# mjoppich/tsxCount

Measured on AMD Instinct MI355X. Metric: k-mers/sec inserted, k=31, 1e9 synthetic k-mers, 1/2/4/8 GPU; --check pass, higher is better.
Workload: dtype u64

## Files before the change

### tsxcount_amd/csrc/tsx_kernels.h

```cpp
#pragma once
#include "tsx_device.h"

namespace tsx {

constexpr int NT = 256;
constexpr int TILE = 4096;
constexpr int HALO = 128;
constexpr int BATCH = 2048;
constexpr int PER_THREAD = BATCH / NT;
constexpr int DSLOTS = 4096;
constexpr int DPROBES = 8;

__device__ __forceinline__ bool is_nl(uint32_t b) { return b == (uint32_t)'\n'; }
__device__ __forceinline__ uint32_t base_code(uint32_t b) { return ((b >> 1) ^ (b >> 2)) & 3u; }

__device__ __forceinline__ void classify16(const uint4 v, bool prev_nl, uint32_t &nl16, uint32_t &le16,
                                           uint32_t &code32) {
    const uint32_t w[4] = {v.x, v.y, v.z, v.w};
    nl16 = 0; code32 = 0;
#pragma unroll
    for (int i = 0; i < 4; ++i) {
        const uint32_t t = ((w[i] >> 1) ^ (w[i] >> 2)) & 0x03030303u;
        const uint32_t x = t | (t >> 6);
        code32 |= ((x | (x >> 12)) & 0xFFu) << (8 * i);
// ... 228 lines not shown
                if (__ballot(valid) == 0ULL) continue;
                uint64_t x[WK];
                extract_kmer<WK>(s_codes, pp, p.top_mask, x);
                uint64_t xp[WK];
#pragma unroll
                for (int t = 0; t < WK; ++t) xp[t] = __shfl_up((unsigned long long)x[t], 1, 64);
                const bool prev_valid = __shfl_up((int)valid, 1, 64) != 0;
                const bool leader = valid && (lane == 0 || !prev_valid || !kmer_eq<WK>(x, xp));
                const unsigned long long bnd = __ballot(leader || !valid);
                const unsigned long long above = (lane == 63) ? 0ULL : (bnd >> (lane + 1));
                const uint32_t runlen = (above ? (uint32_t)__builtin_ctzll(above) : (uint32_t)(63 - lane)) + 1u;
                added += valid ? 1ULL : 0ULL;
                if (leader) {
                    hash_key<CANON, WK>(p, (const uint64_t *)s_lut, x, hk[j]);
                    uint32_t slot = (uint32_t)(mix64(hk[j][0] ^ (WK > 1 ? hk[j][WK - 1] : 0)) >> 40) & (DSLOTS - 1);
                    slot_of[j] = -2; direct_cnt[j] = runlen;
                    for (int pr = 0; pr < DPROBES; ++pr) {
                        const uint32_t old = atomicCAS(&s_dpos[slot], 0u, pp + 1u);
                        if (old == 0u) {
                            atomicAdd(&s_dcnt[slot], runlen);
                            slot_of[j] = (int)slot;
                            break;
                        }
                        uint64_t y[WK];
                        extract_kmer<WK>(s_codes, old - 1u, p.top_mask, y);
                        if (kmer_eq<WK>(x, y)) {
                            atomicAdd(&s_dcnt[slot], runlen);
                            slot_of[j] = -1;
                            break;
                        }
                        slot = (slot + 1) & (DSLOTS - 1);
                    }
                }
            }
            lds_barrier();
#pragma unroll
            for (int j = 0; j < PER_THREAD; ++j) {
                if (slot_of[j] == -1) continue;
                uint64_t d = direct_cnt[j];
                if (slot_of[j] >= 0) {
                    d = s_dcnt[slot_of[j]];
                    s_dcnt[slot_of[j]] = 0;
                    s_dpos[slot_of[j]] = 0;
                }
                insert_key<WK>(p, hk[j], d);
            }
            lds_barrier();
        }
    }
    for (int d = 32; d > 0; d >>= 1) added += __shfl_down(added, d, 64);
    if (lane == 0 && added) atomicAdd(&p.stats[ST_KMERS], added);
}

template <bool HOMOUT = false, bool BR = false>
__global__ __launch_bounds__(NT, 5) void strip_desc_kernel(TableParams p, const uint8_t *buf, uint64_t n, uint64_t own_end,
                                                           int head_open, const uint32_t *tile_line, uint64_t ntiles,
                                                           uint4 *desc, uint64_t desc_cap, unsigned long long *desc_cnt,
                                                           unsigned long long *kmer_sum, int long_desc,
                                                           unsigned long long *hom_out = nullptr,
                                                           const uint16_t *qmap = nullptr) {
    __shared__ uint64_t s_codes[(TILE + HALO) / 32 + 2];
    __shared__ uint64_t s_nl[(TILE + HALO) / 64 + 3];
    __shared__ uint64_t s_le[TILE / 64];
    __shared__ uint8_t s_lb[TILE / 16];
    __shared__ uint32_t s_wsum[NT / 64];
    const int tid = threadIdx.x, lane = tid & 63, wave = tid >> 6;
    if (tid < 3) s_nl[(TILE + HALO) / 64 + tid] = ~0ULL;
    if (tid < 2) s_codes[(TILE + HALO) / 32 + tid] = 0;
    unsigned long long added = 0;
    unsigned long long hacc = 0;
    const uint32_t k = (uint32_t)p.k;
    const uint32_t region = blockIdx.x * (NT / 64) + wave;
    uint4 *my = desc + (uint64_t)region * desc_cap * (long_desc ? 2u : 1u);
    uint32_t fill = 0;
    const uint64_t start_lim = min(own_end, (n >= k) ? n - k + 1 : 0ULL);
    const uint64_t lt = (1ULL << lane) - 1ULL;

    uint4 cur = make_uint4(0x0A0A0A0Au, 0x0A0A0A0Au, 0x0A0A0A0Au, 0x0A0A0A0Au), hcur = cur;
    bool cur_pnl = true;
    uint32_t cur_line = 0;
    if ((uint64_t)blockIdx.x < ntiles) {
        const uint64_t off = (uint64_t)blockIdx.x * TILE + (uint64_t)tid * 16;
        cur_line = tile_line[blockIdx.x];
        cur = load16(buf, off, n);
        cur_pnl = prev_is_nl(buf, off, n, head_open);
        if (tid < HALO / 16) hcur = load16(buf, (uint64_t)blockIdx.x * TILE + TILE + (uint64_t)tid * 16, n);
    }
    for (uint64_t tile = blockIdx.x; tile < ntiles; tile += gridDim.x) {
        const uint64_t base = tile * TILE;
        lds_barrier();
        {
            uint32_t nl, le, code;
            classify16(cur, cur_pnl, nl, le, code);
            if constexpr (BR) nl |= rule_bits16<BR>(p, qmap, cur, base + (uint64_t)tid * 16, n);
            reinterpret_cast<uint32_t *>(s_codes)[tid] = code;
            reinterpret_cast<uint16_t *>(s_nl)[tid] = (uint16_t)nl;
            reinterpret_cast<uint16_t *>(s_le)[tid] = (uint16_t)le;
            if (tid < HALO / 16) {
                uint32_t hnl, hle, hcode;
                classify16(hcur, false, hnl, hle, hcode);
                if constexpr (BR) hnl |= rule_bits16<BR>(p, qmap, hcur, base + TILE + (uint64_t)tid * 16, n);
                reinterpret_cast<uint32_t *>(s_codes)[TILE / 16 + tid] = hcode;
                reinterpret_cast<uint16_t *>(s_nl)[TILE / 16 + tid] = (uint16_t)hnl;
            }
            const uint32_t c = __popc(le);
            const uint32_t inc = wave_incl_scan(c);
            if (lane == 63) s_wsum[wave] = inc;
            lds_barrier();
            uint32_t woff = cur_line;
            for (int w = 0; w < wave; ++w) woff += s_wsum[w];
            s_lb[tid] = (uint8_t)((woff + inc - c) & 3u);
        }
        {
            const uint64_t nt = tile + gridDim.x;
            if (nt < ntiles) {
                const uint64_t off = nt * TILE + (uint64_t)tid * 16;
                cur_line = tile_line[nt];
                cur = load16(buf, off, n);
                cur_pnl = prev_is_nl(buf, off, n, head_open);
                if (tid < HALO / 16) hcur = load16(buf, nt * TILE + TILE + (uint64_t)tid * 16, n);
            }
        }
        lds_barrier();
        const uint32_t s0 = (uint32_t)tid * 16;
        const uint32_t *codes32 = reinterpret_cast<const uint32_t *>(s_codes);
        const uint32_t *nl32 = reinterpret_cast<const uint32_t *>(s_nl);
        uint64_t m;
        {
            const uint32_t w = (uint32_t)tid >> 1, sh = ((uint32_t)tid & 1u) * 16u;
            const uint32_t a0 = nl32[w], a1 = nl32[w + 1], a2 = nl32[w + 2];
            m = (uint64_t)__funnelshift_r(a0, a1, sh) | ((uint64_t)__funnelshift_r(a1, a2, sh) << 32);
        }
        uint64_t r = m;
        uint32_t span = 1;
        while (span * 2 <= k) { r |= r >> span; span *= 2; }
        if (span < k) r |= r >> (k - span);
        const uint32_t e16 = reinterpret_cast<const uint16_t *>(s_le)[tid];
        const uint32_t lb = s_lb[tid];
        uint32_t c0 = e16 << 1; c0 ^= c0 << 1; c0 ^= c0 << 2; c0 ^= c0 << 4; c0 ^= c0 << 8;
        uint32_t c1 = (e16 & c0) << 1; c1 ^= c1 << 1; c1 ^= c1 << 2; c1 ^= c1 << 4; c1 ^= c1 << 8;
        const uint32_t l0 = (lb & 1u) ? 0xFFFFu : 0u, l1 = (lb & 2u) ? 0xFFFFu : 0u;
        const uint32_t b0 = c0 ^ l0, b1 = c1 ^ l1 ^ (c0 & l0);
        const uint64_t g0 = base + s0;
        const uint32_t jmax = (start_lim > g0) ? (uint32_t)min((uint64_t)16, start_lim - g0) : 0u;
        const uint32_t nb1 = (p.line_mask & 2u) ? ~b1 : ~0u;
        uint32_t vm = ~(uint32_t)r & b0 & nb1 & ((1u << jmax) - 1u);
        added += (unsigned long long)__popc(vm);
        if constexpr (HOMOUT) {
            if (vm) {
                const uint32_t c0 = codes32[tid], c1 = codes32[tid + 1], c2 = codes32[tid + 2];
                const uint64_t lo = (uint64_t)c0 | ((uint64_t)c1 << 32), hi = c2;
                const uint64_t xl = lo ^ ((lo >> 2) | (hi << 62)), xh = hi ^ (hi >> 2);
                const uint64_t nl = (xl | (xl >> 1)) & 0x5555555555555555ULL, nh = (xh | (xh >> 1)) & 0x5555555555555555ULL;
                const bool core_ok = ((nl >> 30) & ((1ULL << (2u * (k - 16u))) - 1ULL)) == 0ULL;
              if (core_ok) {
                const uint32_t z = (uint32_t)nl & 0x3FFFFFFFu;
                const uint32_t a = z ? ((31u - (uint32_t)__clz((int)z)) >> 1) + 1u : 0u;
                const uint32_t s2 = 2u * (k - 1u);
                const uint32_t zz = (uint32_t)((nl >> s2) | (nh << (64u - s2))) & 0x3FFFFFFFu;
                const uint32_t b = zz ? (uint32_t)(__ffs((int)zz) - 1) >> 1 : 15u;
                const uint32_t homm = (a <= b) ? (((2u << b) - 1u) & ~((1u << a) - 1u)) & 0xFFFFu : 0u;
                hacc += (unsigned long long)__popc(vm & homm) << (16u * ((c0 >> 30) & 3u));
                vm &= ~homm;
              }
            }
        }
        if (!long_desc) {
            const unsigned long long hb = __ballot(vm != 0u);
            if (hb) {
                const uint32_t nbr = (uint32_t)(((hb << 1) >> lane) & 1ULL) << 16;
                if (vm) my[fill + (uint32_t)__builtin_popcountll(hb & lt)] = make_uint4(codes32[tid], codes32[tid + 1], codes32[tid + 2], vm | nbr);
                fill += (uint32_t)__builtin_popcountll(hb);
            }
        } else {
            const uint32_t v1 = __shfl_down(vm, 1, 64), v2 = __shfl_down(vm, 2, 64), v3 = __shfl_down(vm, 3, 64);
            const uint32_t vlo = vm | (v1 << 16), vhi = v2 | (v3 << 16);
            const bool has = (lane & 3) == 0 && (vlo | vhi) != 0u;
            const unsigned long long hb = __ballot(has);
            if (hb) {
                if (has) {
                    uint4 *o = my + (uint64_t)(fill + (uint32_t)__builtin_popcountll(hb & lt)) * 2u;
                    o[0] = make_uint4(codes32[tid], codes32[tid + 1], codes32[tid + 2], codes32[tid + 3]);
                    o[1] = make_uint4(codes32[tid + 4], codes32[tid + 5], vlo, vhi);
                }
                fill += (uint32_t)__builtin_popcountll(hb);
            }
        }
    }
    for (int d = 32; d > 0; d >>= 1) added += __shfl_down(added, d, 64);
    if (lane == 0) {
        if (added) atomicAdd(&p.stats[ST_KMERS], added);
        if (added && kmer_sum) atomicAdd(kmer_sum, added);
        desc_cnt[region] = fill;
    }
    if constexpr (HOMOUT) {
#pragma unroll
        for (int b = 0; b < 4; ++b) {
            unsigned long long t = (hacc >> (16 * b)) & 0xFFFFULL;
            for (int d = 32; d > 0; d >>= 1) t += __shfl_down(t, d, 64);
            if (lane == 0 && t && hom_out) atomicAdd(&hom_out[b], t);
        }
    }
}

template <bool CANON = false>
__global__ __launch_bounds__(NT, 4) void walk_log_kernel(TableParams p, const uint4 *desc, uint64_t desc_cap,
                                                         const unsigned long long *desc_cnt, uint32_t nregions,
                                                         uint64_t *log, uint64_t log_cap, unsigned long long *log_cnt,
                                                         uint32_t *hist, uint32_t hist_nb, uint32_t hist_shift,
                                                         uint64_t n_packed, int long_desc, int own_only,
                                                         unsigned long long *emit_sum) {
    constexpr int HOT_N = 8;
    __shared__ uint64_t s_hot_key[(NT / 64) * HOT_N];
    __shared__ uint32_t s_hot_cnt[(NT / 64) * HOT_N];
    __shared__ uint32_t s_hist[(NT / 64) * 512];
    __shared__ uint64_t s_roll[CANON ? 128 : 64];
    uint64_t *const s_mroll = s_roll + 64;
    __shared__ uint64_t s_homh[4];
    extern __shared__ uint64_t s_lut[];
    const int tid = threadIdx.x, lane = tid & 63, wave = tid >> 6;
    const int lut_words = p.groups * (1 << p.g);
    for (int i = tid; i < lut_words; i += NT) s_lut[i] = p.lut[i];
    for (int i = tid; i < (NT / 64) * 512; i += NT) s_hist[i] = 0;
    if (tid < 64) s_roll[tid] = p.roll[tid];
    if (CANON && tid < 64) s_mroll[tid] = p.roll[MROLL1_AT + tid];
    if (tid < 4) {
        const uint64_t x[1] = {(0x5555555555555555ULL * (uint64_t)tid) & p.top_mask};
        uint64_t hh[1];
        hash_apply<1>(p, p.lut, x, hh);
        if constexpr (CANON) {
            const uint64_t xc[1] = {(0x5555555555555555ULL * (uint64_t)(3 - tid)) & p.top_mask};
            uint64_t hc[1];
            hash_apply<1>(p, p.lut, xc, hc);
            hh[0] = min(hh[0], hc[0]);
        }
        s_homh[tid] = hh[0];
    }
    if (tid < (NT / 64) * HOT_N) { s_hot_key[tid] = 0; s_hot_cnt[tid] = 0; }
    const uint32_t k = (uint32_t)p.k;
    const uint32_t G = gridDim.x * (NT / 64), region = blockIdx.x * (NT / 64) + wave;
    uint64_t *my_log = log + (uint64_t)region * log_cap;
    uint32_t *my_hist = s_hist + wave * 512;
    uint32_t fill = 0;
    const uint32_t cap32 = (uint32_t)min(log_cap, (uint64_t)0xFFFFFFFFu);
    const TableParams *pk = (const TableParams *)__builtin_amdgcn_kernarg_segment_ptr();
    auto is_mine = [&](uint64_t hk) -> bool {
        if (!own_only) return true;
        const uint64_t h1[1] = {hk};
        return owner_shard<1>(p, h1) == p.shard;
    };
    unsigned long long emitted = 0;
// ... 708 lines not shown
```

### tsxcount_amd/csrc/tsx_partition.h

```cpp
#pragma once
#include "tsx_kernels.h"
#include <type_traits>

namespace tsx {

constexpr int PART_NT = 256;
constexpr int RING_NT = 512;
constexpr int PART_WPT = 4;
constexpr int PART_FLUSH = 16;

template <int RW>
__device__ __forceinline__ void load_rec(const uint64_t *ptr, uint64_t (&r)[RW]) {
    if constexpr (RW == 1) {
        r[0] = *ptr;
    } else {
#pragma unroll
        for (int t = 0; t < RW; t += 2) {
            const uint4 v = *reinterpret_cast<const uint4 *>(ptr + t);
            r[t] = (uint64_t)v.x | ((uint64_t)v.y << 32);
            r[t + 1] = (uint64_t)v.z | ((uint64_t)v.w << 32);
        }
    }
}
template <int RW>
// ... 447 lines not shown
    if ((tid & 63) == 0 && spilled) atomicAdd(&p.stats[ST_FALLBACK], (unsigned long long)spilled);
    if (key_sum) {
        for (int d = 32; d > 0; d >>= 1) ksum += __shfl_down(ksum, d, 64);
        if ((tid & 63) == 0 && ksum) atomicAdd(key_sum, ksum);
    }
}

constexpr int SP_NT = 512;
constexpr uint32_t SP_CAPBITS = 5;

__global__ __launch_bounds__(1024) void desc_prefix_kernel(const unsigned long long *cnt, uint32_t nregions,
                                                           unsigned long long *offs, unsigned long long *total,
                                                           uint64_t desc_cap, uint64_t out_cap, unsigned long long *stats) {
    __shared__ unsigned long long s_w[16];
    const uint32_t tid = threadIdx.x, per = (nregions + 1023u) / 1024u;
    unsigned long long sum = 0, lost = 0;
    for (uint32_t i = 0; i < per; ++i) {
        const uint32_t r = tid * per + i;
        if (r < nregions) { sum += min((unsigned long long)cnt[r], (unsigned long long)desc_cap); lost += cnt[r] > desc_cap ? cnt[r] - desc_cap : 0ULL; }
    }
    const unsigned long long inc = wave_incl_scan64(sum);
    if ((tid & 63) == 63) s_w[tid >> 6] = inc;
    __syncthreads();
    unsigned long long base = inc - sum;
    for (uint32_t w = 0; w < (tid >> 6); ++w) base += s_w[w];
    for (uint32_t i = 0; i < per; ++i) {
        const uint32_t r = tid * per + i;
        if (r < nregions) { offs[r] = base; base += min((unsigned long long)cnt[r], (unsigned long long)desc_cap); }
    }
    if (lost && stats) atomicAdd(&stats[ST_FAIL], lost);
    if (tid == 1023) {
        if (base > out_cap) { if (stats) atomicAdd(&stats[ST_FAIL], base - out_cap); base = out_cap; }
        total[0] = base;
    }
}
__global__ __launch_bounds__(256) void desc_pack_kernel(const uint4 *desc, uint64_t desc_cap, const unsigned long long *cnt,
                                                        const unsigned long long *offs, uint32_t nregions, uint4 *out,
                                                        uint64_t out_cap, uint32_t du) {
    for (uint32_t r = blockIdx.x; r < nregions; r += gridDim.x) {
        const uint64_t n = min((uint64_t)cnt[r], desc_cap) * du, o = offs[r] * du;
        const uint4 *src = desc + (uint64_t)r * desc_cap * du;
        for (uint64_t i = threadIdx.x; i < n; i += 256)
            if (o + i < out_cap) out[o + i] = src[i];
    }
}

template <int NT, bool CANON = false>
__global__ __launch_bounds__(NT, 4) void walk_part_kernel(TableParams p, const uint4 *desc, uint64_t desc_cap,
                                                            const unsigned long long *desc_cnt, uint32_t nregions,
                                                            uint64_t *dst, uint64_t dst_cap, unsigned long long *dst_cnt,
                                                            uint32_t nb, uint32_t shift, uint64_t *ovq_all,
                                                            uint32_t *ovq_cnt, uint32_t ovq_cap, uint64_t n_packed,
                                                            uint32_t dst_g0, uint32_t dst_gtot, int own_flags,
                                                            unsigned long long *emit_sum, int long_desc, uint32_t flush_q) {
    const int own_only = own_flags & 3;
    const bool append = (own_flags & 4) != 0;
    constexpr int HOT_N = 8;
    __shared__ uint64_t s_hot_key[(NT / 64) * HOT_N];
    __shared__ uint32_t s_hot_cnt[(NT / 64) * HOT_N];
    __shared__ uint64_t s_roll[CANON ? 128 : 64];
    __shared__ uint64_t s_lut4[256];
    uint64_t *const s_mroll = s_roll + 64;
    __shared__ uint64_t s_homh[4];
    __shared__ uint32_t s_njobs[2];
    __shared__ uint32_t s_ovn;
    __shared__ uint64_t s_ovk[OVF_N];
    __shared__ uint32_t s_ovc[OVF_N];
    extern __shared__ uint64_t s_part[];
    constexpr uint32_t CAP = 1u << SP_CAPBITS, cmask = CAP - 1;
    uint64_t *s_stage = s_part;
    unsigned long long *s_meta = reinterpret_cast<unsigned long long *>(s_part + ((size_t)nb << SP_CAPBITS));
    unsigned long long *s_th = s_meta + nb;
    uint32_t *s_cur = reinterpret_cast<uint32_t *>(s_th + nb);
    uint32_t *s_job = s_cur + nb;

    const uint32_t tid = threadIdx.x, lane = tid & 63, wave = tid >> 6;
    const uint32_t wg = blockIdx.x;
    const uint32_t cap32 = (uint32_t)min(dst_cap, (uint64_t)0xFFFFFFF0u);
    const uint32_t gl = dst_g0 + wg;
    auto word_of = [&](uint32_t b, uint32_t at) -> uint64_t * { return dst + ((uint64_t)(b * dst_gtot + gl) * (uint64_t)cap32 + at); };
    auto is_mine = [&](uint64_t hk) -> bool {
        if (own_only != 1) return true;
        const uint64_t h1[1] = {hk};
        return owner_shard<1>(p, h1) == p.shard;
    };
    if (tid < 64) s_roll[tid] = p.roll[tid];
    if (tid < 256) s_lut4[tid] = p.roll[64 + tid];
    if (CANON && tid < 64) s_mroll[tid] = p.roll[MROLL1_AT + tid];
    if (tid < 4) {
        const uint64_t x = (0x5555555555555555ULL * (uint64_t)tid) & p.top_mask;
        uint64_t hh = 0;
        for (int grp = 0; grp < 16; ++grp) hh ^= p.roll[64 + grp * 16 + ((x >> (4 * grp)) & 15u)];
        if constexpr (CANON) {
            const uint64_t xc = (0x5555555555555555ULL * (uint64_t)(3 - tid)) & p.top_mask;
            uint64_t hc = 0;
            for (int grp = 0; grp < 16; ++grp) hc ^= p.roll[64 + grp * 16 + ((xc >> (4 * grp)) & 15u)];
            hh = min(hh, hc);
        }
        s_homh[tid] = hh;
    }
    if (tid < (NT / 64) * HOT_N) { s_hot_key[tid] = 0; s_hot_cnt[tid] = 0; }
    if (tid < OVF_N) { s_ovk[tid] = 0; s_ovc[tid] = 0; }
    if (tid < 2) s_njobs[tid] = 0;
    if (tid == 0) s_ovn = (append && ovq_cnt) ? ovq_cnt[blockIdx.x] : 0u;
    for (uint32_t b = tid; b < nb; b += NT) { s_cur[b] = append ? (uint32_t)dst_cnt[(uint64_t)b * dst_gtot + dst_g0 + blockIdx.x] : 0u; s_th[b] = 0; }
    uint64_t *ovq = ovq_all ? ovq_all + (size_t)blockIdx.x * ovq_cap : nullptr;
    unsigned long long added = 0;
    unsigned long long emitted = 0;
    uint32_t spilled = 0;
// ... 77 lines not shown
        }
    };

    lds_barrier();
    for (uint32_t r = blockIdx.x; r < nregions; r += gridDim.x) {
        const uint32_t nr = n_packed ? (uint32_t)(((uint64_t)r * desc_cap < n_packed) ? min(desc_cap, n_packed - (uint64_t)r * desc_cap) : 0ULL)
                                     : (uint32_t)min((uint64_t)desc_cnt[r], desc_cap);
        const uint32_t per = long_desc ? NT / 4 : NT, me = long_desc ? tid >> 2 : tid;
        const uint4 *rd = desc + (uint64_t)r * desc_cap * (long_desc ? 2u : 1u);
        const uint4 z4 = make_uint4(0, 0, 0, 0);
        uint4 dn = z4, dn2 = z4;
        if (me < nr) { if (long_desc) { dn = rd[2u * me]; dn2 = rd[2u * me + 1u]; } else dn = rd[me]; }
        for (uint32_t base = 0; base < nr; base += per) {
            const uint4 d = dn, d2 = dn2;
            if (base + per < nr) {
                dn = z4; dn2 = z4;
                if (base + per + me < nr) {
                    if (long_desc) { dn = rd[2u * (base + per + me)]; dn2 = rd[2u * (base + per + me) + 1u]; }
                    else dn = rd[base + per + me];
                }
            }
            uint32_t cw0 = d.x, cw1 = d.y, cw2 = d.z, vm = d.w & 0xFFFFu;
            if (long_desc) {
                const uint32_t t = tid & 3u;
                const uint32_t w0 = d.x, w1 = d.y, w2 = d.z, w3 = d.w, w4 = d2.x, w5 = d2.y;
                cw0 = (t == 0u) ? w0 : (t == 1u) ? w1 : (t == 2u) ? w2 : w3;
                cw1 = (t == 0u) ? w1 : (t == 1u) ? w2 : (t == 2u) ? w3 : w4;
                cw2 = (t == 0u) ? w2 : (t == 1u) ? w3 : (t == 2u) ? w4 : w5;
                const uint32_t vw = (t < 2u) ? d2.z : d2.w;
                vm = (vw >> ((t & 1u) * 16u)) & 0xFFFFu;
            }
            const bool wave_has = __ballot(vm != 0u) != 0ULL;
            uint64_t h = 0, hr = 0;
            uint32_t inc = 0, single = 0;
            if (wave_has) {
                const uint64_t lo = (uint64_t)cw0 | ((uint64_t)cw1 << 32), hi = cw2;
                if (vm) {
                    const uint64_t x = lo & p.top_mask;
                    for (uint32_t grp = 0; grp < ngrp; ++grp) h ^= s_lut4[grp * 16u + ((uint32_t)(x >> (4u * grp)) & 15u)];
                    if constexpr (CANON) {
                        const uint64_t xa[1] = {x};
                        uint64_t r[1];
                        revcomp<1>(xa, p.n, r);
                        for (uint32_t grp = 0; grp < ngrp; ++grp) hr ^= s_lut4[grp * 16u + ((uint32_t)(r[0] >> (4u * grp)) & 15u)];
                    }
                }
                {
                    const uint32_t o = 2u * k, ws = o >> 5, sh = o & 31u;
                    const uint32_t w0 = (ws == 0u) ? cw0 : (ws == 1u) ? cw1 : cw2;
                    const uint32_t w1 = (ws == 0u) ? cw1 : (ws == 1u) ? cw2 : 0u;
                    inc = __funnelshift_r(w0, w1, sh);
                }
            uint32_t homm = 0;
            if (own_only != 2) {
                const uint64_t dlo = lo ^ ((lo >> 2) | (hi << 62)), dhi = hi ^ (hi >> 2);
                uint64_t rlo = (dlo | (dlo >> 1)) & 0x5555555555555555ULL, rhi = (dhi | (dhi >> 1)) & 0x5555555555555555ULL;
                uint32_t span = 1;
                while (span * 2 <= k - 1) {
                    const uint32_t sh = 2u * span;
                    rlo |= (rlo >> sh) | (rhi << (64u - sh));
                    rhi |= rhi >> sh;
                    span *= 2;
                }
                if (span < k - 1) {
                    const uint32_t sh = 2u * (k - 1 - span);
                    rlo |= (rlo >> sh) | (rhi << (64u - sh));
                }
                uint32_t x = ~(uint32_t)rlo & 0x55555555u;
                x = (x | (x >> 1)) & 0x33333333u;
                x = (x | (x >> 2)) & 0x0F0F0F0Fu;
                x = (x | (x >> 4)) & 0x00FF00FFu;
                homm = (x | (x >> 8)) & 0xFFFFu;
            }
            const uint32_t hv = vm & homm;
            single = vm & ~homm;
            if (__ballot(hv != 0u)) {
                for (uint32_t b = 0; b < 4; ++b) {
                    uint32_t e = cw0 ^ (0x55555555u * b);
                    uint32_t y = ~(e | (e >> 1)) & 0x55555555u;
                    y = (y | (y >> 1)) & 0x33333333u;
                    y = (y | (y >> 2)) & 0x0F0F0F0Fu;
                    y = (y | (y >> 4)) & 0x00FF00FFu;
                    y = (y | (y >> 8)) & 0xFFFFu;
                    uint32_t tot = (uint32_t)__popc(hv & y);
                    if (__ballot(tot != 0u) == 0ULL) continue;
                    for (int d = 32; d > 0; d >>= 1) tot += __shfl_xor(tot, d, 64);
                    if (lane == 0 && is_mine(s_homh[b])) {
                        emitted += tot;
                        const uint64_t key = s_homh[b];
                        uint64_t *hkey = s_hot_key + wave * HOT_N;
                        uint32_t *hcnt = s_hot_cnt + wave * HOT_N;
                        int at = -1;
                        for (int q = 0; q < HOT_N; ++q)
                            if (hcnt[q] && hkey[q] == key) { at = q; break; }
                        if (at < 0)
                            for (int q = 0; q < HOT_N; ++q)
                                if (!hcnt[q]) { at = q; hkey[q] = key; break; }
                        if (at >= 0 && (uint64_t)hcnt[at] + tot < 0xFFFFFFF0ULL) hcnt[at] += tot;
                        else defer_append1(pk, key, tot);
                    }
                }
            }
        }
            bool waited = false;
            for (uint32_t j0 = 0; j0 < 16; j0 += 4) {
                const uint32_t s4 = (single >> j0) & 0xFu;
                if (wave_has) {
// ... 6 lines not shown
                                                 (__builtin_amdgcn_ubfe(inc, 2u * (j0 + j), 2u) << 4);
                            if constexpr (CANON) hr = mirror_step(p, s_mroll, hr, idx);
                            h = (h >> 2) ^ s_roll[idx];
                        }
                    }
                    uint32_t m4 = s4;
                    if (own_only) {
                        if (own_only == 1) {
#pragma unroll
                            for (int j = 0; j < 4; ++j)
                                if (((s4 >> j) & 1u) && !is_mine(hs[j])) m4 &= ~(1u << j);
                        }
                        emitted += (unsigned long long)__popc(m4);
                    }
                    if (__ballot(m4 != 0u) != 0ULL) {
                        uint32_t bq[4];
                        unsigned long long sl[4];
#pragma unroll
                        for (int j = 0; j < 4; ++j) {
                            bq[j] = (uint32_t)(hs[j] >> shift) & (nb - 1);
                            sl[j] = ((m4 >> j) & 1u) ? atomicAdd(&s_th[bq[j]], 1ULL) : 0ULL;
                        }
#pragma unroll
                        for (int j = 0; j < 4; ++j) {
                            if ((m4 >> j) & 1u) {
                                const uint32_t b = bq[j];
                                if ((uint32_t)sl[j] - (uint32_t)(sl[j] >> 32) < CAP) {
                                    s_stage[(b << SP_CAPBITS) + (((uint32_t)sl[j] ^ b) & cmask)] = hs[j];
                                } else {
                                    const uint32_t at = atomicAdd(&s_cur[b], 1u);
                                    if (at < cap32) *word_of(b, at) = hs[j];
                                    else spill(hs[j]);
                                }
                            }
                        }
                    }
                }
                if ((((j0 >> 2) + 1u) % flush_q) == 0u) {
                    lds_barrier();
                    flush(false, !waited);
                    waited = true;
                    lds_barrier();
                }
            }
        }
    }
    lds_barrier();
    flush(true, false);
    lds_barrier();
    for (uint32_t b = tid; b < nb; b += NT) dst_cnt[(uint64_t)b * dst_gtot + gl] = min(s_cur[b], cap32);
    if (tid < OVF_N && s_ovc[tid]) defer_append1(pk, s_ovk[tid] ^ OVF_SALT, s_ovc[tid]);
    if (tid == 0 && ovq_cnt) ovq_cnt[blockIdx.x] = min(s_ovn, ovq_cap);
    if (tid < (NT / 64) * HOT_N && s_hot_cnt[tid]) defer_append1(pk, s_hot_key[tid], s_hot_cnt[tid]);
    if (emit_sum) {
        for (int d = 32; d > 0; d >>= 1) emitted += __shfl_down(emitted, d, 64);
        if (lane == 0 && emitted) atomicAdd(emit_sum, emitted);
    }
    for (int d = 32; d > 0; d >>= 1) { added += __shfl_down(added, d, 64); spilled += __shfl_down(spilled, d, 64); }
    if (lane == 0) {
        if (added) atomicAdd(&p.stats[ST_KMERS], added);
        if (spilled) atomicAdd(&p.stats[ST_FALLBACK], (unsigned long long)spilled);
    }
}

template <int WK>
__global__ __launch_bounds__(PART_NT) void overflow_insert_kernel(TableParams p, const uint64_t *ovq_all,
                                                                  const uint32_t *ovq_cnt, uint32_t cap, uint32_t nq) {
    constexpr int RW = RecWords<WK>::value;
    for (uint32_t qi = blockIdx.x; qi < nq; qi += gridDim.x) {
        const uint32_t n = ovq_cnt[qi];
        for (uint32_t i = threadIdx.x; i < n; i += PART_NT) {
            uint64_t h[WK];
#pragma unroll
            for (int t = 0; t < WK; ++t) h[t] = ovq_all[((size_t)qi * cap + i) * RW + t];
            insert_key<WK>(p, h, 1);
        }
    }
}

template <int WK>
__global__ __launch_bounds__(PART_NT) void deferred_insert_kernel(TableParams p, const uint64_t *rec, const uint64_t *cnt,
                                                                  const unsigned long long *n_ptr, uint64_t n_fixed,
                                                                  uint64_t cap) {
    constexpr int RW = RecWords<WK>::value;
    const uint64_t n = min(n_ptr ? (uint64_t)*n_ptr : n_fixed, cap);
    constexpr uint32_t DN = (RW == 1) ? 2048u : (RW == 2) ? 1024u : 512u;
    __shared__ uint64_t s_k[DN * RW];
    __shared__ unsigned long long s_c[DN];
    __shared__ uint32_t s_r[(RW > 1) ? DN : 1];
    for (uint32_t t = threadIdx.x; t < DN; t += PART_NT) { s_k[t * RW] = 0; s_c[t] = 0; if (RW > 1) s_r[t] = 0; }
    __syncthreads();
    const uint64_t per = (n + gridDim.x - 1) / gridDim.x;
    const uint64_t lo = min(n, (uint64_t)blockIdx.x * per), hi = min(n, lo + per);
    for (uint64_t i = lo + threadIdx.x; i < hi; i += PART_NT) {
        const uint64_t d = cnt ? cnt[i] : 1ULL;
        if (d == 0) continue;
        uint64_t h[WK];
#pragma unroll
        for (int t = 0; t < WK; ++t) h[t] = rec[i * RW + t];
        if (p.lg != p.l && owner_shard<WK>(p, h) != p.shard) continue;
        const uint64_t kk = h[0] ^ OVF_SALT;
        uint64_t mixin = h[0];
#pragma unroll
        for (int t = 1; t < WK; ++t) mixin ^= h[t] * 0x9E3779B97F4A7C15ULL;
        uint32_t slot = (uint32_t)(mix64(mixin) >> 40) & (DN - 1);
        bool done = false;
// ... 587 lines not shown
```

### tsxcount_amd/csrc/tsxcount_hip.hip

```cpp
#include "../../include/tsxcount_hip.h"
#include "tsx_kernels.h"
#include "tsx_partition.h"
#include "tsx_minimizer.h"
#include "tsx_inflate.h"
#include "tsx_output.h"
#include "tsx_query.h"
#include "tsx_baserule.h"
#include "tsx_db.h"
#include "tsx_combine.h"
#include "tsx_fasta.h"

#include <mutex>
#include <hip/hip_runtime.h>

#include <algorithm>
#include <cstdio>
#include <cstdlib>
#include <cerrno>
#include <cmath>
#include <cstring>
#include <deque>
#include <string>
#include <thread>
#include <vector>
// ... 958 lines not shown
    unsigned long long *counts = nullptr, *key_sum = nullptr;
};

struct DescOut { uint4 *out = nullptr; uint64_t cap = 0; unsigned long long *count = nullptr, *sum = nullptr; int long_desc = 0; int owners = 0; };

static int run_fastq_piece(tsx_hip_map *m, const uint8_t *d_text, uint64_t n, uint64_t own_end, int head_open,
                           hipStream_t st, ShardOut sh = ShardOut(), HotOut hot = HotOut(), DescOut dsc = DescOut()) {
    uint64_t *shard_send = sh.send;
    const uint64_t shard_cap = sh.send_cap;
    unsigned long long *shard_counts = sh.counts;
    if (own_end == 0) return TSX_HIP_OK;
    const uint64_t ntiles = (own_end + TILE - 1) / TILE;
    if (ntiles > m->tile_cap) {
        if (m->d_tile) { HIP_TRY(hipStreamSynchronize(st)); HIP_TRY(hipFree(m->d_tile)); m->d_tile = nullptr; }
        m->tile_cap = ntiles + ntiles / 4 + 1024;
        HIP_TRY(hipMalloc((void **)&m->d_tile, (m->tile_cap + m->tile_cap / SCAN_CHUNK + 16) * sizeof(uint32_t)));
    }
    hipEvent_t *ev = nullptr;
    if (m->timing) {
        if (m->ev_used + EV_N > m->ev.size()) {
            for (int i = 0; i < EV_N; ++i) { hipEvent_t e; HIP_TRY(hipEventCreate(&e)); m->ev.push_back(e); }
        }
        ev = &m->ev[m->ev_used]; m->ev_used += EV_N;
        HIP_TRY(hipEventRecord(ev[0], st));
    }
    const int g1 = (int)std::min<uint64_t>(ntiles, (uint64_t)m->cus * 8);
    hipLaunchKernelGGL(line_count_kernel, dim3(g1), dim3(NT), 0, st, d_text, n, own_end, head_open, m->d_tile, ntiles);
    {
        const uint64_t nchunks = (ntiles + SCAN_CHUNK - 1) / SCAN_CHUNK;
        uint32_t *chunk = m->d_tile + m->tile_cap;
        hipLaunchKernelGGL(line_chunk_sum_kernel, dim3((uint32_t)nchunks), dim3(SCAN_CHUNK), 0, st,
                           (const uint32_t *)m->d_tile, ntiles, chunk);
        hipLaunchKernelGGL(line_chunk_scan_kernel, dim3(1), dim3(1024), 0, st, chunk, nchunks, m->d_carry);
        hipLaunchKernelGGL(line_scan_kernel, dim3((uint32_t)nchunks), dim3(SCAN_CHUNK), 0, st, m->d_tile, ntiles,
                           (const uint32_t *)chunk);
    }
    if (ev) HIP_TRY(hipEventRecord(ev[1], st));
    if (dsc.out || dsc.owners) {
        const int gdd = (int)std::min<uint64_t>(ntiles, (uint64_t)m->cus * 8), gdr = gdd * (NT / 64);
        const uint32_t du = dsc.long_desc ? 2u : 1u;
        const uint64_t dcap = ((ntiles + gdd - 1) / gdd) * (dsc.long_desc ? 16 : 64);
        int rcd = grow(st, m->d_buf[1], m->buf_bytes[1], (size_t)gdr * dcap * du * 16);
        if (rcd != TSX_HIP_OK) return rcd;
        {
            size_t have = m->desc_cnt_entries;
            rcd = grow(st, m->d_desc_cnt, have, ((size_t)2 * gdr + 16) * 8 + (size_t)MZ_MAX_RANKS * m->cus * MZ_WG_PER_CU * 4 + 64);
            m->desc_cnt_entries = have;
            if (rcd != TSX_HIP_OK) return rcd;
        }
        unsigned long long *d_cnt = m->d_desc_cnt, *d_offs = d_cnt + gdr, *d_tot = d_offs + gdr;
        if (dsc.owners) {
            unsigned long long *d_hom = d_cnt + 2 * (size_t)gdr + 8 + ((size_t)MZ_MAX_RANKS * m->cus * MZ_WG_PER_CU + 1) / 2;
            HIP_TRY(hipMemsetAsync(d_hom, 0, 32, st));
            hipLaunchKernelGGL(strip_desc_kernel<true>, dim3(gdd), dim3(NT), 0, st, m->p, d_text, n, own_end, head_open,
                               (const uint32_t *)m->d_tile, ntiles, (uint4 *)m->d_buf[1], dcap, d_cnt, dsc.sum, 0, d_hom);
        } else
        DISPATCH_BR(m, hipLaunchKernelGGL((strip_desc_kernel<false, BRV>), dim3(gdd), dim3(NT), 0, st, m->p, d_text, n, own_end,
                           head_open, (const uint32_t *)m->d_tile, ntiles, (uint4 *)m->d_buf[1], dcap, d_cnt, dsc.sum,
                           dsc.long_desc, (unsigned long long *)nullptr, m->qmap_cur));
        if (dsc.owners) {
            HIP_TRY(hipGetLastError());
            m->mz_regions = (uint32_t)gdr; m->mz_dcap = dcap;
            if (ev) {
                for (int i = 2; i < EV_N; ++i) HIP_TRY(hipEventRecord(ev[i], st));
                m->ev_open.push_back((long)(ev - m->ev.data()));
            }
            return TSX_HIP_OK;
        }
        hipLaunchKernelGGL(desc_prefix_kernel, dim3(1), dim3(1024), 0, st, (const unsigned long long *)d_cnt, (uint32_t)gdr,
                           d_offs, d_tot, dcap, (uint64_t)dsc.cap, m->p.stats);
        hipLaunchKernelGGL(desc_pack_kernel, dim3(std::min(gdr, m->cus * 8)), dim3(256), 0, st, (const uint4 *)m->d_buf[1], dcap,
                           (const unsigned long long *)d_cnt, (const unsigned long long *)d_offs, (uint32_t)gdr, dsc.out,
                           dsc.cap * du, du);
        HIP_TRY(hipGetLastError());
        HIP_TRY(hipMemcpyAsync(dsc.count, d_tot, 8, hipMemcpyDeviceToDevice, st));
        if (ev) {
            for (int i = 2; i < EV_N; ++i) HIP_TRY(hipEventRecord(ev[i], st));
            m->ev_open.push_back((long)(ev - m->ev.data()));
        }
        return TSX_HIP_OK;
    }
    const size_t lut_bytes = m->lut.size() * 8;
    const int g3 = (int)std::min<uint64_t>(ntiles, (uint64_t)m->cus * 3);

    const TableParams &p = m->p;
    const bool use_part = shard_send || (can_partition(m) && !slab_bits(m) &&
                                         (m->path == 2 || (m->path == 0 && own_end * 32 >= m->lay.table_bytes)));
    if (!use_part) {
        int rcz = ensure_zeroed(m, st);
        if (rcz != TSX_HIP_OK) return rcz;
        DISPATCH_BR(m, DISPATCH_CANON(m, DISPATCH_WK(m, hipLaunchKernelGGL((count_fastq_kernel<WKV, CANV, BRV>), dim3(g3), dim3(NT),
                                                            lut_bytes, st, m->p, d_text, n, own_end, head_open,
                                                            (const uint32_t *)m->d_tile, ntiles, m->qmap_cur))));
        HIP_TRY(hipGetLastError());
        if (ev) for (int i = 2; i < EV_N; ++i) HIP_TRY(hipEventRecord(ev[i], st));
        return TSX_HIP_OK;
    }

    const uint64_t maxrec = (p.line_mask == 3 ? own_end / 2 : own_end) + 65536;
    const uint32_t nown = 1u << (p.lg - p.l);
    const int scan_wgs = (p.wk == 1) ? SCAN_WG_PER_CU : (p.wk == 2 ? 6 : 3);
    const int gs = (int)std::min<uint64_t>(ntiles, (uint64_t)m->cus * scan_wgs);
    const int greg = gs * (NT / 64);
    PartPlan pl;
    const char *fuse_env = getenv("TSX_HIP_FUSE");
    const int fuse = (fuse_env && atoi(fuse_env) == 0) ? 0 : 2;
    const int g_sp = (int)std::min<uint64_t>((own_end + 8191) / 8192, (uint64_t)m->cus * 2);
    const int desc_wgs = 8;
    const int gd = (int)std::min<uint64_t>(ntiles, (uint64_t)m->cus * desc_wgs), gdreg = gd * (NT / 64);
    const bool want_fuse = fuse && !shard_send && p.wk == 1;

    int rc = plan_partition(m, maxrec, (want_fuse && fuse == 2) ? std::max(greg, gdreg) : greg, true, shard_send ? nown : 0, st,
                            pl, want_fuse ? g_sp : 0);
    if (rc == TSX_HIP_OK && want_fuse && !pl.fused)
        rc = plan_partition(m, maxrec, greg, true, 0, st, pl, 0);
    if (rc != TSX_HIP_OK) return rc;
    TableParams pp = m->p;
    if (shard_send) {
        pp.defer = DeferList{hot.keys, hot.cnts, hot.n, hot.cap};
    } else {
        rc = ensure_deferred(m, maxrec, st);
        if (rc != TSX_HIP_OK) return rc;
        HIP_TRY(hipMemsetAsync(m->d_def_n, 0, 8, st));
        pp.defer = DeferList{m->d_def_rec, m->d_def_cnt, m->d_def_n, (uint64_t)m->def_cap};
    }
    const uint32_t hist_nb = shard_send ? nown : pl.nb1, hist_shift = (uint32_t)(shard_send ? p.l : p.l - pl.b1);
    if (pl.fused) {
        const uint32_t nq2 = pl.nb1 * pl.cpr2;
        rc = ensure_ovq(m, (size_t)nq2 + pl.G1, pl.rw, st);
        if (rc != TSX_HIP_OK) return rc;
        const size_t lds = (size_t)pl.nb1 * (((size_t)8 << SP_CAPBITS) + 8 + 8 + 4 + 4);
        {
            const char *ll_env = getenv("TSX_HIP_LOCAL_LONG");
            const int lng = ll_env ? (atoi(ll_env) != 0) : 0;
            const uint64_t desc_cap = ((ntiles + gd - 1) / gd) * (lng ? 16 : 64);
            rc = grow(st, m->d_buf[0], m->buf_bytes[0], (size_t)gdreg * desc_cap * (lng ? 32 : 16));
            if (rc != TSX_HIP_OK) return rc;
            DISPATCH_BR(m, hipLaunchKernelGGL((strip_desc_kernel<false, BRV>), dim3(gd), dim3(NT), 0, st, pp, d_text, n, own_end,
                               head_open, (const uint32_t *)m->d_tile, ntiles, (uint4 *)m->d_buf[0], desc_cap, pl.c_log,
                               (unsigned long long *)nullptr, lng, (unsigned long long *)nullptr, m->qmap_cur));
            HIP_TRY(hipGetLastError());
            if (lds > ((size_t)80 << 10)) {
                DISPATCH_CANON(m, hipLaunchKernelGGL((walk_part_kernel<1024, CANV>), dim3(pl.G1), dim3(1024), lds, st, pp,
                                   (const uint4 *)m->d_buf[0], desc_cap,
                                   (const unsigned long long *)pl.c_log, (uint32_t)gdreg, pl.buf1, pl.cap1, pl.c_l1, pl.nb1,
                                   (uint32_t)(p.l - pl.b1), m->d_ovq + (size_t)nq2 * OVQ_CAP, m->d_ovq_cnt + nq2, OVQ_CAP,
                                   (uint64_t)0, 0u, pl.G1, 0, (unsigned long long *)nullptr, lng, 1u));
            } else {
                DISPATCH_CANON(m, hipLaunchKernelGGL((walk_part_kernel<SP_NT, CANV>), dim3(pl.G1), dim3(SP_NT), lds, st, pp,
                                   (const uint4 *)m->d_buf[0], desc_cap,
                                   (const unsigned long long *)pl.c_log, (uint32_t)gdreg, pl.buf1, pl.cap1, pl.c_l1, pl.nb1,
                                   (uint32_t)(p.l - pl.b1), m->d_ovq + (size_t)nq2 * OVQ_CAP, m->d_ovq_cnt + nq2, OVQ_CAP,
                                   (uint64_t)0, 0u, pl.G1, 0, (unsigned long long *)nullptr, lng, 1u));
            }
        }
    } else if (p.wk == 1) {
        const uint64_t desc_cap = ((ntiles + gd - 1) / gd) * 64;
        rc = grow(st, m->d_buf[1], m->buf_bytes[1], (size_t)gdreg * desc_cap * 16);
        if (rc != TSX_HIP_OK) return rc;
        pl.buf1 = m->d_buf[1];
        {
            size_t have = m->desc_cnt_entries;
            rc = grow(st, m->d_desc_cnt, have, (size_t)gdreg * 8);
            m->desc_cnt_entries = have;
            if (rc != TSX_HIP_OK) return rc;
        }
        DISPATCH_BR(m, hipLaunchKernelGGL((strip_desc_kernel<false, BRV>), dim3(gd), dim3(NT), 0, st, pp, d_text, n, own_end,
                           head_open, (const uint32_t *)m->d_tile, ntiles, (uint4 *)m->d_buf[1], desc_cap, m->d_desc_cnt,
                           (unsigned long long *)nullptr, 0, (unsigned long long *)nullptr, m->qmap_cur));
        HIP_TRY(hipGetLastError());
        DISPATCH_CANON(m, hipLaunchKernelGGL((walk_log_kernel<CANV>), dim3(gs), dim3(NT), lut_bytes, st, pp,
                           (const uint4 *)m->d_buf[1], desc_cap,
                           (const unsigned long long *)m->d_desc_cnt, (uint32_t)gdreg, m->d_buf[0], pl.log_cap,
                           pl.c_log, pl.d_hist, hist_nb, hist_shift, (uint64_t)0, 0, 0, (unsigned long long *)nullptr));
    } else {
        const int du = (2 * p.wk + 2 + 3) / 4;
        const uint64_t desc_cap = ((ntiles + gd - 1) / gd) * 64;
        rc = grow(st, m->d_buf[1], m->buf_bytes[1], (size_t)gdreg * desc_cap * du * 16);
        if (rc != TSX_HIP_OK) return rc;
        pl.buf1 = m->d_buf[1];
        {
            size_t have = m->desc_cnt_entries;
            rc = grow(st, m->d_desc_cnt, have, (size_t)gdreg * 8);
            m->desc_cnt_entries = have;
            if (rc != TSX_HIP_OK) return rc;
        }
#define TSX_WIDE2(WKV)                                                                                                      \
        DISPATCH_BR(m, hipLaunchKernelGGL((strip_desc_wide_kernel<WKV, BRV>), dim3(gd), dim3(NT), 0, st, pp, d_text, n,      \
                           own_end, head_open, (const uint32_t *)m->d_tile, ntiles, (uint4 *)m->d_buf[1], desc_cap,         \
                           m->d_desc_cnt, m->qmap_cur));                                                                     \
        DISPATCH_CANON(m, hipLaunchKernelGGL((walk_log_wide_kernel<WKV, CANV>), dim3(gs), dim3(NT), lut_bytes, st, pp,     \
                           (const uint4 *)m->d_buf[1],                                                                       \
                           desc_cap, (const unsigned long long *)m->d_desc_cnt, (uint32_t)gdreg, m->d_buf[0],                \
                           pl.log_cap, pl.c_log, pl.d_hist, hist_nb, hist_shift))
        switch (p.wk) {
            case 2: TSX_WIDE2(2); break;
            case 3: TSX_WIDE2(3); break;
            default: TSX_WIDE2(4); break;
        }
#undef TSX_WIDE2
    }
    HIP_TRY(hipGetLastError());
    if (ev) { HIP_TRY(hipEventRecord(ev[2], st)); HIP_TRY(hipEventRecord(ev[3], st)); }
    if (shard_send) {
        if ((uint64_t)greg * pl.log_cap > shard_cap || (sh.own && (uint64_t)greg * pl.log_cap > sh.own_cap))
            return TSX_HIP_ERANGE;
        hipLaunchKernelGGL(offsets_rows_kernel, dim3(nown), dim3(1024), 0, st, (const uint32_t *)pl.d_hist, pl.d_offs,
                           (uint32_t)greg, pl.c_bcnt);
        hipLaunchKernelGGL(offsets_finish_kernel, dim3(1), dim3(1024), 0, st, nown, pl.c_bstart, pl.c_bcnt);
        hipLaunchKernelGGL(split_owner_kernel, dim3(std::min(greg, m->cus * 8)), dim3(PART_NT), 0, st,
                           (const uint64_t *)m->d_buf[0], (const unsigned long long *)pl.c_log, pl.log_cap,
                           (uint32_t)greg, shard_send, (const unsigned long long *)pl.d_offs,
                           (const unsigned long long *)pl.c_bstart, (const unsigned long long *)pl.c_bcnt, nown,
                           (uint32_t)p.l, sh.own, p.shard, sh.key_sum);
        HIP_TRY(hipGetLastError());
        HIP_TRY(hipMemcpyAsync(shard_counts, pl.c_bcnt, nown * sizeof(unsigned long long), hipMemcpyDeviceToDevice, st));
    } else {
        rc = run_partition_build(m, pl, m->d_buf[0], nullptr, pl.log_cap, st, ev);
        if (rc != TSX_HIP_OK) return rc;
    }
// ... 2704 lines not shown
```

Before: 82.80 billion.

## Strip homopolymer k-mers in descriptor kernel and count them directly in walk

Extends the descriptor-producing strip kernel so that, on the partitioned walk path, homopolymer k-mers are detected and removed from the descriptor masks. Their counts are accumulated per base and added once through the deferred list by block 0 of the walk kernel. A new mode handles k<16 using window masks. The walk kernel can then skip its own homopolymer detection (flag 8). Per-base accumulators are split into four 32-bit counters instead of one packed 64-bit value, which avoids 16-bit overflow. This cuts descriptor writes and hot-key contention for repetitive k-mers, at the cost of extra ALU work in the strip kernel and a reused slot in the deferred-count buffer.

```diff
diff --git a/tsxcount_amd/csrc/tsx_kernels.h b/tsxcount_amd/csrc/tsx_kernels.h
--- a/tsxcount_amd/csrc/tsx_kernels.h
+++ b/tsxcount_amd/csrc/tsx_kernels.h
@@ -304,7 +304,7 @@
     if (lane == 0 && added) atomicAdd(&p.stats[ST_KMERS], added);
 }
 
-template <bool HOMOUT = false, bool BR = false>
+template <int HOMOUT = 0, bool BR = false>
 __global__ __launch_bounds__(NT, 5) void strip_desc_kernel(TableParams p, const uint8_t *buf, uint64_t n, uint64_t own_end,
                                                            int head_open, const uint32_t *tile_line, uint64_t ntiles,
                                                            uint4 *desc, uint64_t desc_cap, unsigned long long *desc_cnt,
@@ -320,13 +320,15 @@
     if (tid < 3) s_nl[(TILE + HALO) / 64 + tid] = ~0ULL;
     if (tid < 2) s_codes[(TILE + HALO) / 32 + tid] = 0;
     unsigned long long added = 0;
-    unsigned long long hacc = 0;
+    uint32_t hacc0 = 0, hacc1 = 0, hacc2 = 0, hacc3 = 0;
     const uint32_t k = (uint32_t)p.k;
     const uint32_t region = blockIdx.x * (NT / 64) + wave;
     uint4 *my = desc + (uint64_t)region * desc_cap * (long_desc ? 2u : 1u);
     uint32_t fill = 0;
     const uint64_t start_lim = min(own_end, (n >= k) ? n - k + 1 : 0ULL);
     const uint64_t lt = (1ULL << lane) - 1ULL;
+    [[maybe_unused]] const uint64_t wh_lo = (k + 14u >= 32u) ? ~0ULL : ((1ULL << (2u * (k + 14u))) - 1ULL);
+    [[maybe_unused]] const uint64_t wh_hi = (k > 18u) ? ((1ULL << (2u * (k - 18u))) - 1ULL) : 0ULL;
 
     uint4 cur = make_uint4(0x0A0A0A0Au, 0x0A0A0A0Au, 0x0A0A0A0Au, 0x0A0A0A0Au), hcur = cur;
     bool cur_pnl = true;
@@ -398,23 +400,34 @@
         const uint32_t nb1 = (p.line_mask & 2u) ? ~b1 : ~0u;
         uint32_t vm = ~(uint32_t)r & b0 & nb1 & ((1u << jmax) - 1u);
         added += (unsigned long long)__popc(vm);
-        if constexpr (HOMOUT) {
+        if constexpr (HOMOUT != 0) {
             if (vm) {
                 const uint32_t c0 = codes32[tid], c1 = codes32[tid + 1], c2 = codes32[tid + 2];
                 const uint64_t lo = (uint64_t)c0 | ((uint64_t)c1 << 32), hi = c2;
                 const uint64_t xl = lo ^ ((lo >> 2) | (hi << 62)), xh = hi ^ (hi >> 2);
                 const uint64_t nl = (xl | (xl >> 1)) & 0x5555555555555555ULL, nh = (xh | (xh >> 1)) & 0x5555555555555555ULL;
-                const bool core_ok = ((nl >> 30) & ((1ULL << (2u * (k - 16u))) - 1ULL)) == 0ULL;
-              if (core_ok) {
-                const uint32_t z = (uint32_t)nl & 0x3FFFFFFFu;
-                const uint32_t a = z ? ((31u - (uint32_t)__clz((int)z)) >> 1) + 1u : 0u;
-                const uint32_t s2 = 2u * (k - 1u);
-                const uint32_t zz = (uint32_t)((nl >> s2) | (nh << (64u - s2))) & 0x3FFFFFFFu;
-                const uint32_t b = zz ? (uint32_t)(__ffs((int)zz) - 1) >> 1 : 15u;
-                const uint32_t homm = (a <= b) ? (((2u << b) - 1u) & ~((1u << a) - 1u)) & 0xFFFFu : 0u;
-                hacc += (unsigned long long)__popc(vm & homm) << (16u * ((c0 >> 30) & 3u));
-                vm &= ~homm;
-              }
+                uint32_t hv = 0, hb = 0;
+                if constexpr (HOMOUT == 1) {
+                    const bool core_ok = ((nl >> 30) & ((1ULL << (2u * (k - 16u))) - 1ULL)) == 0ULL;
+                    if (core_ok) {
+                        const uint32_t z = (uint32_t)nl & 0x3FFFFFFFu;
+                        const uint32_t a = z ? ((31u - (uint32_t)__clz((int)z)) >> 1) + 1u : 0u;
+                        const uint32_t s2 = 2u * (k - 1u);
+                        const uint32_t zz = (uint32_t)((nl >> s2) | (nh << (64u - s2))) & 0x3FFFFFFFu;
+                        const uint32_t b = zz ? (uint32_t)(__ffs((int)zz) - 1) >> 1 : 15u;
+                        const uint32_t homm = (a <= b) ? (((2u << b) - 1u) & ~((1u << a) - 1u)) & 0xFFFFu : 0u;
+                        hv = vm & homm;
+                        hb = (c0 >> 30) & 3u;
+                    }
+                } else {
+                    if (((nl & wh_lo) | (nh & wh_hi)) == 0ULL) { hv = vm; hb = c0 & 3u; }
+                }
+                if (hv) {
+                    const uint32_t pc = (uint32_t)__popc(hv);
+                    hacc0 += (hb == 0u) ? pc : 0u; hacc1 += (hb == 1u) ? pc : 0u;
+                    hacc2 += (hb == 2u) ? pc : 0u; hacc3 += (hb == 3u) ? pc : 0u;
+                    vm &= ~hv;
+                }
             }
         }
         if (!long_desc) {
@@ -445,10 +458,11 @@
         if (added && kmer_sum) atomicAdd(kmer_sum, added);
         desc_cnt[region] = fill;
     }
-    if constexpr (HOMOUT) {
+    if constexpr (HOMOUT != 0) {
+        const uint32_t hl[4] = {hacc0, hacc1, hacc2, hacc3};
 #pragma unroll
         for (int b = 0; b < 4; ++b) {
-            unsigned long long t = (hacc >> (16 * b)) & 0xFFFFULL;
+            unsigned long long t = hl[b];
             for (int d = 32; d > 0; d >>= 1) t += __shfl_down(t, d, 64);
             if (lane == 0 && t && hom_out) atomicAdd(&hom_out[b], t);
         }
diff --git a/tsxcount_amd/csrc/tsx_partition.h b/tsxcount_amd/csrc/tsx_partition.h
--- a/tsxcount_amd/csrc/tsx_partition.h
+++ b/tsxcount_amd/csrc/tsx_partition.h
@@ -523,9 +523,11 @@
                                                             uint32_t nb, uint32_t shift, uint64_t *ovq_all,
                                                             uint32_t *ovq_cnt, uint32_t ovq_cap, uint64_t n_packed,
                                                             uint32_t dst_g0, uint32_t dst_gtot, int own_flags,
-                                                            unsigned long long *emit_sum, int long_desc, uint32_t flush_q) {
+                                                            unsigned long long *emit_sum, int long_desc, uint32_t flush_q,
+                                                            const unsigned long long *hom_in = nullptr) {
     const int own_only = own_flags & 3;
     const bool append = (own_flags & 4) != 0;
+    const bool hom_gone = own_only == 2 || (own_flags & 8) != 0;
     constexpr int HOT_N = 8;
     __shared__ uint64_t s_hot_key[(NT / 64) * HOT_N];
     __shared__ uint32_t s_hot_cnt[(NT / 64) * HOT_N];
@@ -709,7 +711,7 @@
                     inc = __funnelshift_r(w0, w1, sh);
                 }
             uint32_t homm = 0;
-            if (own_only != 2) {
+            if (!hom_gone) {
                 const uint64_t dlo = lo ^ ((lo >> 2) | (hi << 62)), dhi = hi ^ (hi >> 2);
                 uint64_t rlo = (dlo | (dlo >> 1)) & 0x5555555555555555ULL, rhi = (dhi | (dhi >> 1)) & 0x5555555555555555ULL;
                 uint32_t span = 1;
@@ -822,6 +824,7 @@
     if (tid < OVF_N && s_ovc[tid]) defer_append1(pk, s_ovk[tid] ^ OVF_SALT, s_ovc[tid]);
     if (tid == 0 && ovq_cnt) ovq_cnt[blockIdx.x] = min(s_ovn, ovq_cap);
     if (tid < (NT / 64) * HOT_N && s_hot_cnt[tid]) defer_append1(pk, s_hot_key[tid], s_hot_cnt[tid]);
+    if (hom_in && blockIdx.x == 0 && tid < 4 && hom_in[tid]) defer_append1(pk, s_homh[tid], hom_in[tid]);
     if (emit_sum) {
         for (int d = 32; d > 0; d >>= 1) emitted += __shfl_down(emitted, d, 64);
         if (lane == 0 && emitted) atomicAdd(emit_sum, emitted);
diff --git a/tsxcount_amd/csrc/tsxcount_hip.hip b/tsxcount_amd/csrc/tsxcount_hip.hip
--- a/tsxcount_amd/csrc/tsxcount_hip.hip
+++ b/tsxcount_amd/csrc/tsxcount_hip.hip
@@ -1034,10 +1034,10 @@
         if (dsc.owners) {
             unsigned long long *d_hom = d_cnt + 2 * (size_t)gdr + 8 + ((size_t)MZ_MAX_RANKS * m->cus * MZ_WG_PER_CU + 1) / 2;
             HIP_TRY(hipMemsetAsync(d_hom, 0, 32, st));
-            hipLaunchKernelGGL(strip_desc_kernel<true>, dim3(gdd), dim3(NT), 0, st, m->p, d_text, n, own_end, head_open,
+            hipLaunchKernelGGL(strip_desc_kernel<1>, dim3(gdd), dim3(NT), 0, st, m->p, d_text, n, own_end, head_open,
                                (const uint32_t *)m->d_tile, ntiles, (uint4 *)m->d_buf[1], dcap, d_cnt, dsc.sum, 0, d_hom);
         } else
-        DISPATCH_BR(m, hipLaunchKernelGGL((strip_desc_kernel<false, BRV>), dim3(gdd), dim3(NT), 0, st, m->p, d_text, n, own_end,
+        DISPATCH_BR(m, hipLaunchKernelGGL((strip_desc_kernel<0, BRV>), dim3(gdd), dim3(NT), 0, st, m->p, d_text, n, own_end,
                            head_open, (const uint32_t *)m->d_tile, ntiles, (uint4 *)m->d_buf[1], dcap, d_cnt, dsc.sum,
                            dsc.long_desc, (unsigned long long *)nullptr, m->qmap_cur));
         if (dsc.owners) {
@@ -1103,7 +1103,7 @@
     } else {
         rc = ensure_deferred(m, maxrec, st);
         if (rc != TSX_HIP_OK) return rc;
-        HIP_TRY(hipMemsetAsync(m->d_def_n, 0, 8, st));
+        HIP_TRY(hipMemsetAsync(m->d_def_n, 0, 8 + 32, st));
         pp.defer = DeferList{m->d_def_rec, m->d_def_cnt, m->d_def_n, (uint64_t)m->def_cap};
     }
     const uint32_t hist_nb = shard_send ? nown : pl.nb1, hist_shift = (uint32_t)(shard_send ? p.l : p.l - pl.b1);
@@ -1118,22 +1118,36 @@
             const uint64_t desc_cap = ((ntiles + gd - 1) / gd) * (lng ? 16 : 64);
             rc = grow(st, m->d_buf[0], m->buf_bytes[0], (size_t)gdreg * desc_cap * (lng ? 32 : 16));
             if (rc != TSX_HIP_OK) return rc;
-            DISPATCH_BR(m, hipLaunchKernelGGL((strip_desc_kernel<false, BRV>), dim3(gd), dim3(NT), 0, st, pp, d_text, n, own_end,
-                               head_open, (const uint32_t *)m->d_tile, ntiles, (uint4 *)m->d_buf[0], desc_cap, pl.c_log,
-                               (unsigned long long *)nullptr, lng, (unsigned long long *)nullptr, m->qmap_cur));
+            int hom = (p.k >= 16) ? 1 : 2;
+            if (const char *e = getenv("TSX_HIP_HOM_STRIPS")) { const int v = atoi(e); if (v == 0 || v == 2 || (v == 1 && p.k >= 16)) hom = v; }
+            if (lng) hom = 0;
+            unsigned long long *d_hom = hom ? m->d_def_n + 1 : nullptr;
+            const int wflags = (hom == 1) ? 8 : 0;
+#define TSX_DESC(HOMV)                                                                                                       \
+            DISPATCH_BR(m, hipLaunchKernelGGL((strip_desc_kernel<HOMV, BRV>), dim3(gd), dim3(NT), 0, st, pp, d_text, n, own_end,  \
+                               head_open, (const uint32_t *)m->d_tile, ntiles, (uint4 *)m->d_buf[0], desc_cap, pl.c_log,     \
+                               (unsigned long long *)nullptr, lng, d_hom, m->qmap_cur))
+            switch (hom) {
+                case 1: TSX_DESC(1); break;
+                case 2: TSX_DESC(2); break;
+                default: TSX_DESC(0); break;
+            }
+#undef TSX_DESC
             HIP_TRY(hipGetLastError());
             if (lds > ((size_t)80 << 10)) {
                 DISPATCH_CANON(m, hipLaunchKernelGGL((walk_part_kernel<1024, CANV>), dim3(pl.G1), dim3(1024), lds, st, pp,
                                    (const uint4 *)m->d_buf[0], desc_cap,
                                    (const unsigned long long *)pl.c_log, (uint32_t)gdreg, pl.buf1, pl.cap1, pl.c_l1, pl.nb1,
                                    (uint32_t)(p.l - pl.b1), m->d_ovq + (size_t)nq2 * OVQ_CAP, m->d_ovq_cnt + nq2, OVQ_CAP,
-                                   (uint64_t)0, 0u, pl.G1, 0, (unsigned long long *)nullptr, lng, 1u));
+                                   (uint64_t)0, 0u, pl.G1, wflags, (unsigned long long *)nullptr, lng, 1u,
+                                   (const unsigned long long *)d_hom));
             } else {
                 DISPATCH_CANON(m, hipLaunchKernelGGL((walk_part_kernel<SP_NT, CANV>), dim3(pl.G1), dim3(SP_NT), lds, st, pp,
                                    (const uint4 *)m->d_buf[0], desc_cap,
                                    (const unsigned long long *)pl.c_log, (uint32_t)gdreg, pl.buf1, pl.cap1, pl.c_l1, pl.nb1,
                                    (uint32_t)(p.l - pl.b1), m->d_ovq + (size_t)nq2 * OVQ_CAP, m->d_ovq_cnt + nq2, OVQ_CAP,
-                                   (uint64_t)0, 0u, pl.G1, 0, (unsigned long long *)nullptr, lng, 1u));
+                                   (uint64_t)0, 0u, pl.G1, wflags, (unsigned long long *)nullptr, lng, 1u,
+                                   (const unsigned long long *)d_hom));
             }
         }
     } else if (p.wk == 1) {
@@ -1147,7 +1161,7 @@
             m->desc_cnt_entries = have;
             if (rc != TSX_HIP_OK) return rc;
         }
-        DISPATCH_BR(m, hipLaunchKernelGGL((strip_desc_kernel<false, BRV>), dim3(gd), dim3(NT), 0, st, pp, d_text, n, own_end,
+        DISPATCH_BR(m, hipLaunchKernelGGL((strip_desc_kernel<0, BRV>), dim3(gd), dim3(NT), 0, st, pp, d_text, n, own_end,
                            head_open, (const uint32_t *)m->d_tile, ntiles, (uint4 *)m->d_buf[1], desc_cap, m->d_desc_cnt,
                            (unsigned long long *)nullptr, 0, (unsigned long long *)nullptr, m->qmap_cur));
         HIP_TRY(hipGetLastError());
```

New measurement: 83.68 billion, median of 6. +1.1%, better.
